# GEOS-ESM/QuickChem

Measured on NVIDIA B200. Metric: OH grid-cell predictions/sec, higher is better.
Workload: dtype f32

## Files before the change

### quickchem_b200/csrc/capi_xgb.cpp

```cpp
#include "context.hpp"

#include <condition_variable>
#include <mutex>
#ifdef __linux__
#include <sched.h>
#endif
#if defined(__x86_64__)
#include <emmintrin.h>
#endif

using namespace qcoh;

namespace qcoh {
template <class T>
static cudaTextureObject_t linear_texture(T *p, size_t n) {
  cudaResourceDesc rd;
  memset(&rd, 0, sizeof rd);
  rd.resType = cudaResourceTypeLinear;
  rd.res.linear.devPtr = p;
  rd.res.linear.desc = cudaCreateChannelDesc<T>();
  rd.res.linear.sizeInBytes = n * sizeof(T);
  cudaTextureDesc td;
  memset(&td, 0, sizeof td);
  td.readMode = cudaReadModeElementType;
  cudaTextureObject_t t = 0;
  CU(cudaCreateTextureObject(&t, &rd, &td, nullptr));
  return t;
}

void upload(Booster *b) {
  if (b->uploaded) return;
  if (!b->loaded) throw Error("Booster has no model: call XGBoosterLoadModel first");
  ensure_device();
  const FlatForest &f = b->flat;
  const size_t nn = (size_t)f.num_nodes();
  {
    std::vector<uint32_t> dev_nodes(f.nodes_xy);
    for (size_t i = 0; i < nn; ++i) {
      if ((dev_nodes[2 * i + 1] & kMetaRelMask) == 0) continue;
      float thr;
      memcpy(&thr, &dev_nodes[2 * i], 4);
      if (std::isnan(thr)) throw Error("split threshold is NaN (node " + std::to_string(i) + ")");
      dev_nodes[2 * i] = neg_threshold_key(thr);
    }
    CU(cudaMemcpy(b->d_nodes.need(nn), dev_nodes.data(), nn * 8, cudaMemcpyHostToDevice));
    b->dev_nodes_host = std::move(dev_nodes);
  }
  CU(cudaMemcpy(b->d_off.need(f.tree_offset.size()), f.tree_offset.data(), f.tree_offset.size() * 4, cudaMemcpyHostToDevice));
  {
    std::vector<int32_t> dd(f.tree_depth.size());
    for (size_t i = 0; i < dd.size(); ++i) {
      if (f.tree_depth[i] > 255) throw Error("tree " + std::to_string(i) + " is deeper than 255 levels");
      dd[i] = f.tree_depth[i] | (std::min(f.tree_min_leaf_depth[i], 255) << 8);
    }
    CU(cudaMemcpy(b->d_depth.need(dd.size()), dd.data(), dd.size() * 4, cudaMemcpyHostToDevice));
  }
  CU(cudaMemcpy(b->d_orig.need(nn), f.orig_id.data(), nn * 4, cudaMemcpyHostToDevice));
  if (b->dev.tex) cudaDestroyTextureObject(b->dev.tex);
  if (b->dev.tex4) cudaDestroyTextureObject(b->dev.tex4);
  b->dev = DeviceForest();
  b->dev.nodes = b->d_nodes.p, b->dev.tree_offset = b->d_off.p, b->dev.tree_depth = b->d_depth.p, b->dev.orig_id = b->d_orig.p;
  b->dev.ntree = (int32_t)b->host.trees.size();
  b->dev.nfeat = (int32_t)b->host.num_feature;
  b->dev.base_score = b->host.base_score;
  if (nn > 0 && nn < ((size_t)1 << 27)) b->dev.tex = linear_texture(b->d_nodes.p, nn);
  if (b->duo.ok && b->duo.num_slots() > 0 && b->duo.num_slots() < ((int64_t)1 << 27)) {
    const size_t ns = (size_t)b->duo.num_slots();
    CU(cudaMemcpy(b->d_recs.need(ns), b->duo.rec.data(), ns * 16, cudaMemcpyHostToDevice));
    b->dev.tex4 = linear_texture(b->d_recs.p, ns);
    b->dev.recs = b->d_recs.p;
    b->dev.duo_has_dl = b->duo.has_default_bits ? 1 : 0;
    b->dev.duo_shallow = (int64_t)ns * 16 < kShallowRecBytesPerTree * std::max<int64_t>(1, b->dev.ntree) ? 1 : 0;
    b->dev.duo_blk_mul = 1u << (32 - b->duo.blk_shift);
  }
  b->uploaded = true;
}

static thread_local struct {
  uint64_t owner = 0;
  ConstWindow w;
} g_const;

ConstWindow hold(Booster *b, int tree0, int ntree) {
  if (ntree <= 0 || ntree > kConstTreesMax || tree0 + ntree > b->dev.ntree) return {};
  int w0 = tree0 - tree0 % kConstTreesMax;
  if (tree0 + ntree > w0 + kConstTreesMax) w0 = tree0;
  const int n = std::min(b->dev.ntree - w0, kConstTreesMax);
  auto held = [&](TopLayout l) { return g_const.owner == b->version && g_const.w.holds(l, tree0, tree0 + ntree); };
  auto fill = [&](TopLayout l) {
    g_const.owner = 0;
    const cudaError_t e = l == TopLayout::kRecordTops
                              ? upload_const_duo(b->duo.top_xy.data() + (size_t)w0 * (2u << kDuoTop), b->duo.tree_slot.data() + w0, n, g.stream)
                              : upload_const_top(b->dev_nodes_host.data(), b->flat.tree_offset.data() + w0, n, g.stream);
    if (e != cudaSuccess) {
      (void)cudaGetLastError();
      return false;
    }
    g_const.owner = b->version, g_const.w = ConstWindow{l, w0, n};
    return true;
  };
  const bool records = b->dev.recs != nullptr && b->dev.tex != 0 && g.duo != 0;
  if (records && (held(TopLayout::kRecordTops) || fill(TopLayout::kRecordTops))) return g_const.w;
  if (held(TopLayout::kNodeTops) || fill(TopLayout::kNodeTops)) return g_const.w;
  return {};
}

void launch_predict_chunked(Booster *b, PredictArgs a, cudaStream_t s) {
  const int t_end = a.tree_end;
  if (a.nrow == 0) return;
  if (t_end <= 0) {
    if (!a.pred_leaf) {
      float v = b->host.base_score;
      if (a.exp10) v = (float)exp10((double)v) * a.scale;
      CU(launch_fill(a.out, a.nrow, v, s));
    }
    return;
  }
  for (int t0 = 0; t0 < t_end; t0 += kRangeTrees) {
    const int n = std::min(kRangeTrees, t_end - t0);
    const ConstWindow w = hold(b, t0, n);
    PredictArgs c = a;
    c.tree_begin = t0, c.tree_end = t0 + n;
    c.first = t0 == 0, c.last = t0 + n == t_end;
    CU(launch_predict(b->dev, w, c, s));
  }
}

static void seal(DMatrix *d) {
  ensure_device();
  int *fl = d->flags.need(1);
  CU(cudaMemsetAsync(fl, 0, sizeof(int), g.stream));
  if (g_spare_Xt.cap >= tile_words(d->nrow, d->ncol) && g_spare_Xt.p && !d->Xt.p) d->Xt.swap(g_spare_Xt);
  CU(launch_seal_tiles(d->X.p, d->nrow, (int)d->ncol, d->missing, d->Xt.need(tile_words(d->nrow, d->ncol)), fl, g.stream));
  CU(cudaMemcpyAsync(&d->hflags, fl, sizeof(int), cudaMemcpyDeviceToHost, g.stream));
  CU(cudaStreamSynchronize(g.stream));
  d->sealed = true;
  if (d->hflags & 2) throw Error("Check failed: valid: Input data contains `inf` or `nan`");
}

static unsigned trees_used(const Booster *b, unsigned ntree_limit) {
  const unsigned nt = (unsigned)b->host.trees.size();
  return (ntree_limit == 0 || ntree_limit > nt) ? nt : ntree_limit;
}

static void predict_into(Booster *b, DMatrix *d, int option_mask, unsigned ntree_limit, const qcoh_epilogue *epi, float *out_dev) {
  upload(b);
  if (!d->sealed) seal(d);
  if (option_mask & ~3) throw Error("option_mask " + std::to_string(option_mask) + ": only 0 (value), 1 (margin) and 2 (leaf index) are supported");
  if (d->ncol > b->host.num_feature)
    throw Error("Check failed: Number of columns does not match number of features in booster. Columns: " +
                std::to_string(d->ncol) + " Features: " + std::to_string(b->host.num_feature));
  PredictArgs a;
  a.Xt = d->Xt.p, a.nrow = d->nrow, a.ncol = (int32_t)d->ncol;
// ... 826 lines not shown
```

### quickchem_b200/csrc/context.hpp

```cpp
#pragma once
#include <cuda_runtime.h>
#include <nvtx3/nvToolsExt.h>

#include <algorithm>
#include <cmath>
#include <cstdio>
#include <cstdlib>
#include <cstring>
#include <memory>
#include <mutex>
#include <stdexcept>
#include <string>
#include <thread>
#include <unordered_set>
#include <utility>
#include <vector>

#include "../../include/qcoh.h"
#include "forest.hpp"
#include "kernels.hpp"

namespace qcoh {

inline thread_local std::string g_err;
// ... 99 lines not shown
}

template <class T>
struct DevBuf {
  T *p = nullptr;
  size_t cap = 0;
  T *need(size_t n) {
    if (n > cap) {
      if (p) cudaFree(p);
      p = nullptr, cap = 0;
      CU(cudaMalloc((void **)&p, (n ? n : 1) * sizeof(T)));
      cap = n;
    }
    return p;
  }
  void release() {
    if (p) cudaFree(p);
    p = nullptr, cap = 0;
  }
  void swap(DevBuf &o) {
    std::swap(p, o.p);
    std::swap(cap, o.cap);
  }
  DevBuf() = default;
  DevBuf(const DevBuf &) = delete;
  DevBuf &operator=(const DevBuf &) = delete;
  ~DevBuf() { release(); }
};

template <class T>
struct PinBuf {
  T *p = nullptr;
  size_t cap = 0;
  T *need(size_t n) {
    if (n > cap) {
      if (p) cudaFreeHost(p);
      p = nullptr, cap = 0;
      CU(cudaHostAlloc((void **)&p, (n ? n : 1) * sizeof(T), cudaHostAllocDefault));
      cap = n;
    }
    return p;
  }
  void swap(PinBuf &o) {
    std::swap(p, o.p);
    std::swap(cap, o.cap);
  }
  PinBuf() = default;
  PinBuf(const PinBuf &) = delete;
  PinBuf &operator=(const PinBuf &) = delete;
  ~PinBuf() {
    if (p) cudaFreeHost(p);
  }
};

inline bool is_device_ptr(const void *p) {
  cudaPointerAttributes a;
  cudaError_t e = cudaPointerGetAttributes(&a, p);
  if (e != cudaSuccess) {
    (void)cudaGetLastError();
    return false;
  }
  return a.type == cudaMemoryTypeDevice || a.type == cudaMemoryTypeManaged;
}

constexpr uint32_t kBoosterMagic = 0x51434253;
constexpr uint32_t kDMatrixMagic = 0x5143444d;
constexpr uint32_t kOhMagic = 0x51434f48;

inline thread_local std::unordered_set<const void *> g_live_handles;
inline bool is_live(const void *h) { return h && g_live_handles.count(h) != 0; }

struct Booster {
  uint32_t magic = kBoosterMagic;
  int oh_refs = 0;
  uint64_t version = 0;
  bool loaded = false, uploaded = false;
  bool cache_owned = false;
  HostForest host;
  FlatForest flat;
  std::vector<uint32_t> dev_nodes_host;
  DeviceForest dev;
  DuoForest duo;
  DevBuf<uint4> d_recs;
  DevBuf<uint2> d_nodes;
  DevBuf<uint32_t> d_off;
  DevBuf<int32_t> d_depth, d_orig;
  DevBuf<float> d_result;
  PinBuf<float> h_result;
  std::vector<bst_ulong> h_shape;
  ShapForest shap;
  bool shap_uploaded = false;
  DevBuf<uint4> d_shap_bins;
  DevBuf<float> d_shap_mean;
  DevBuf<double> d_shap_part;
  Booster() = default;
  Booster(const Booster &) = delete;
  Booster &operator=(const Booster &) = delete;
  ~Booster() {
    if (dev.tex) cudaDestroyTextureObject(dev.tex);
    if (dev.tex4) cudaDestroyTextureObject(dev.tex4);
  }
};

struct DMatrix {
  uint32_t magic = kDMatrixMagic;
  uint64_t nrow = 0, ncol = 0;
  float missing = NAN;
  DevBuf<float> X;
  DevBuf<uint32_t> Xt;
  DevBuf<int> flags;
  int hflags = 1;
  bool sealed = false;
  const void *spec_booster = nullptr;
  uint64_t spec_version = 0;
  bool spec_ready = false;
  DevBuf<float> spec_dev;
  PinBuf<float> spec_host;
};

inline thread_local DevBuf<float> g_spare_X;
inline thread_local DevBuf<uint32_t> g_spare_Xt;
inline thread_local PinBuf<float> g_spare_pin;
inline thread_local DevBuf<float> g_spare_spec;
inline thread_local DevBuf<int> g_chunk_flags;
inline thread_local PinBuf<int> g_h_chunk_flags;
inline thread_local Booster *g_last_booster = nullptr;
inline thread_local uint64_t g_version_counter = 0;

inline Booster *B(BoosterHandle h) {
  Booster *b = (Booster *)h;
  if (!b || !is_live(h) || b->magic != kBoosterMagic) throw Error("Invalid booster handle");
  return b;
}
inline DMatrix *D(DMatrixHandle h) {
  DMatrix *d = (DMatrix *)h;
  if (!d || !is_live(h) || d->magic != kDMatrixMagic) throw Error("Invalid DMatrix handle");
  return d;
}

void upload(Booster *b);
ConstWindow hold(Booster *b, int tree0, int ntree);
void launch_predict_chunked(Booster *b, PredictArgs a, cudaStream_t s);
const ShapForest &shap_tables(Booster *b);

}
```

### quickchem_b200/csrc/forest.hpp

```cpp
#pragma once
#include <cstdint>
#include <cstring>
#include <string>
#include <vector>

namespace qcoh {

struct HostTree {
  std::vector<int32_t> cleft, cright, parent;
  std::vector<uint32_t> sindex;
  std::vector<float> info;
  std::vector<float> loss_chg, sum_hess, base_weight;
  std::vector<int32_t> leaf_child_cnt;
  int32_t num_nodes() const { return (int32_t)cleft.size(); }
};

enum ModelFormat { kLegacyBinary = 0, kJson = 1, kUbjson = 2 };

struct HostForest {
  float base_score = 0.5f;
  uint32_t num_feature = 0;
  uint32_t version[3] = {1, 6, 0};
  std::string objective = "reg:squarederror";
  std::vector<HostTree> trees;
  std::vector<int32_t> tree_info;
  std::vector<std::pair<std::string, std::string>> attributes;
  ModelFormat format = kLegacyBinary;
};

constexpr uint32_t kMetaFeatShift = 26;
constexpr uint32_t kMetaDefaultLeftBit = 1u << 23;
constexpr uint32_t kMetaRelMask = (1u << 23) - 1;
constexpr uint32_t kMaxFeatures = 31;

struct FlatForest {
  std::vector<uint32_t> nodes_xy;
  std::vector<uint32_t> tree_offset;
  std::vector<int32_t> tree_depth;
  std::vector<int32_t> tree_min_leaf_depth;
  std::vector<int32_t> orig_id;
  int32_t max_depth = 0;
  int64_t num_nodes() const { return (int64_t)orig_id.size(); }
};

inline uint32_t neg_threshold_key(float thr) {
  thr += 0.0f;
  uint32_t bits;
  memcpy(&bits, &thr, 4);
  return 0u - (bits ^ ((bits >> 31) ? 0xFFFFFFFFu : 0x80000000u));
}

constexpr int kDuoTop = 4;
constexpr uint32_t kDuoDlRoot = 1u << 17, kDuoDlLeft = 1u << 16, kDuoDlRight = 1u << 15;
constexpr uint32_t kTopDefaultLeftBit = 1u;
struct DuoForest {
  bool ok = false;
  std::string why;
  int blk_shift = 18;
  bool has_default_bits = true;
  std::vector<uint32_t> rec;
  std::vector<uint32_t> tree_slot;
  std::vector<uint32_t> top_xy;
  int64_t num_slots() const { return (int64_t)(rec.size() / 4); }
};
DuoForest build_duo(const struct FlatForest &f, uint32_t num_feature);

constexpr uint32_t kShapNoFeature = 0xFF;
struct ShapForest {
  bool ok = false;
  std::vector<float> mean;
  std::vector<uint32_t> bins;
  std::vector<int64_t> tree_bin;
  int32_t max_path_len = 0;
  int64_t num_paths = 0, num_elements = 0;
  int64_t num_bins() const { return (int64_t)(bins.size() / 128); }
};
ShapForest build_shap(const struct HostForest &h, const struct FlatForest &f);
float shap_bias(const ShapForest &s, const struct HostForest &h, const struct FlatForest &f, int ntree);

struct PredictConfig {
  int type = 0;
  bool training = false;
  int64_t iteration_begin = 0, iteration_end = 0;
  bool strict_shape = false;
};
PredictConfig parse_predict_config(const char *json);

HostForest load_model_file(const std::string &path);
HostForest load_model_buffer(const unsigned char *buf, size_t len);
void save_model_file(const HostForest &f, const std::string &path);
FlatForest flatten(const HostForest &f);

}
```

### quickchem_b200/csrc/kernels.cu

```cuda
#include "kernels.hpp"

#include <cfloat>
#include <cmath>
#include <cstring>
#include <vector>

#include "forest.hpp"

namespace qcoh {

static thread_local uint64_t g_launches = 0;
uint64_t launch_count() { return g_launches; }

#define QC_LAUNCHED() (++g_launches, cudaGetLastError())

namespace {
enum Family { kDuo, kNodes8 = kDuo + 4, kSoaDuo = kNodes8 + 4, kSoaNodes8, kSealTiles, kShap, kShapReduce, kShapApprox, kFamilies };
const char *const kFamilyName[kFamilies] = {"duo", "duo_missing", "duo_leaf", "duo_missing_leaf", "nodes8", "nodes8_missing",
                                            "nodes8_leaf", "nodes8_missing_leaf", "soa_duo", "soa_nodes8", "seal_tiles",
                                            "shap", "shap_reduce", "shap_approx"};
thread_local uint64_t g_family[kFamilies];
thread_local const char *g_last_predict = "";
void count_family(int f) { ++g_family[f]; }
void count_predict(int f) { ++g_family[f], g_last_predict = kFamilyName[f]; }
}
uint64_t kernel_launches(const char *family) {
  for (int i = 0; i < kFamilies; ++i)
    if (!strcmp(kFamilyName[i], family)) return g_family[i];
  return 0;
}
const char *last_predict_kernel() { return g_last_predict; }

__global__ void fill_kernel(float *p, uint64_t n, float v) {
  const uint64_t stride = (uint64_t)gridDim.x * blockDim.x;
  for (uint64_t i = (uint64_t)blockIdx.x * blockDim.x + threadIdx.x; i < n; i += stride) p[i] = v;
}
cudaError_t launch_fill(float *p, uint64_t n, float v, cudaStream_t s) {
  if (n == 0) return cudaSuccess;
  int blocks = (int)((n + 255) / 256 < 148 * 16 ? (n + 255) / 256 : 148 * 16);
  fill_kernel<<<blocks, 256, 0, s>>>(p, n, v);
  return QC_LAUNCHED();
}

constexpr int kBlock = kTileRows;
constexpr int kStride = kTileRows;
static_assert(kStride * 4 == 1024, "the address arithmetic of the walks assumes a 1 KB feature stride");

constexpr uint32_t kKeyMissing = 0xFFFFFFFFu;
__device__ __forceinline__ uint32_t float_key(float v) {
  const uint32_t b = __float_as_uint(__fadd_rn(v, 0.0f));
  return b ^ ((uint32_t)((int32_t)b >> 31) | 0x80000000u);
}
__device__ __forceinline__ uint32_t step_index(uint32_t idx, uint32_t rel, uint32_t x, uint32_t kv) {
  asm("{\n\t.reg .u32 t;\n\tadd.cc.u32 t, %2, %3;\n\taddc.u32 %0, %0, %1;\n\t}" : "+r"(idx) : "r"(rel), "r"(x), "r"(kv));
  return idx;
}
__device__ __forceinline__ uint32_t add_carry_out(uint32_t a, uint32_t b) {
  uint32_t c;
  asm("{\n\t.reg .u32 t;\n\tadd.cc.u32 t, %1, %2;\n\taddc.u32 %0, 0, 0;\n\t}" : "=r"(c) : "r"(a), "r"(b));
  return c;
}
__device__ __forceinline__ uint32_t lds_u32(uint32_t saddr) {
  uint32_t v;
  asm volatile("ld.shared.u32 %0, [%1];" : "=r"(v) : "r"(saddr));
  return v;
}

constexpr int kConstTopNodes = kConstTreesMax << kDuoTop;
__constant__ uint2 c_top[kConstTopNodes];
__constant__ uint32_t c_duo_base[kConstTreesMax];

cudaError_t upload_const_top(const uint32_t *dev_nodes_xy, const uint32_t *tree_offset, int ntree, cudaStream_t s) {
  constexpr int stride = 1 << kDuoTop;
  if (ntree > kConstTreesMax) return cudaErrorInvalidValue;
  std::vector<uint2> host((size_t)ntree * stride);
  for (int t = 0; t < ntree; ++t) {
    const uint32_t n0 = tree_offset[t], n1 = tree_offset[t + 1];
    for (int i = 0; i < stride; ++i) {
      const uint32_t n = n0 + (uint32_t)i;
      host[t * stride + i] = n < n1 ? make_uint2(dev_nodes_xy[2 * n], dev_nodes_xy[2 * n + 1]) : make_uint2(0u, 0u);
    }
  }
  return cudaMemcpyToSymbolAsync(c_top, host.data(), sizeof(uint2) * (size_t)ntree * stride, 0, cudaMemcpyHostToDevice, s);
}

cudaError_t upload_const_duo(const uint32_t *top_xy, const uint32_t *tree_slot, int ntree, cudaStream_t s) {
  if (ntree > kConstTreesMax) return cudaErrorInvalidValue;
  cudaError_t e = cudaMemcpyToSymbolAsync(c_top, top_xy, sizeof(uint2) * ((size_t)ntree << kDuoTop), 0, cudaMemcpyHostToDevice, s);
  if (e != cudaSuccess) return e;
  return cudaMemcpyToSymbolAsync(c_duo_base, tree_slot, sizeof(uint32_t) * (size_t)ntree, 0, cudaMemcpyHostToDevice, s);
}

__device__ __forceinline__ void mbar_init(uint32_t bar, uint32_t count) {
  asm volatile("mbarrier.init.shared::cta.b64 [%0], %1;" ::"r"(bar), "r"(count));
}
__device__ __forceinline__ void mbar_init_fence() { asm volatile("fence.mbarrier_init.release.cluster;" ::: "memory"); }
__device__ __forceinline__ void mbar_expect_tx(uint32_t bar, uint32_t bytes) {
  asm volatile("mbarrier.arrive.expect_tx.shared::cta.b64 _, [%0], %1;" ::"r"(bar), "r"(bytes) : "memory");
}
__device__ __forceinline__ void bulk_g2s(uint32_t dst, const void *src, uint32_t bytes, uint32_t bar) {
  asm volatile("cp.async.bulk.shared::cluster.global.mbarrier::complete_tx::bytes [%0], [%1], %2, [%3];" ::"r"(dst),
               "l"(src), "r"(bytes), "r"(bar)
               : "memory");
}
__device__ __forceinline__ void mbar_wait(uint32_t bar, uint32_t parity) {
  asm volatile(
      "{\n"
      ".reg .pred p;\n"
      "WAIT_%=:\n"
      "mbarrier.try_wait.parity.shared::cta.b64 p, [%0], %1;\n"
      "@p bra DONE_%=;\n"
      "bra WAIT_%=;\n"
      "DONE_%=:\n"
      "}\n" ::"r"(bar),
      "r"(parity)
      : "memory");
}

struct TilePipe {
  uint32_t smem0, bar0, tile_bytes, src_skip, dst_skip;
  const uint32_t *Xt;
  uint64_t ntile, tile, tile_stride;
  uint32_t it;
  __device__ __forceinline__ void issue(uint64_t t) const {
    mbar_expect_tx(bar0, tile_bytes);
    if (tile_bytes) bulk_g2s(smem0 + dst_skip, Xt + t * tile_stride + src_skip, tile_bytes, bar0);
  }
  __device__ __forceinline__ void begin(uint32_t *smem, unsigned long long *bar, const PredictArgs &a, int nfeat, bool with_order, int tid) {
    smem0 = (uint32_t)__cvta_generic_to_shared(smem), bar0 = (uint32_t)__cvta_generic_to_shared(bar);
    tile_stride = (uint64_t)(a.ncol + 1) * kStride;
    tile_bytes = (uint32_t)(a.ncol + (with_order ? 1 : 0)) * kStride * 4u;
    src_skip = with_order ? 0u : (uint32_t)kStride, dst_skip = with_order ? 0u : (uint32_t)kStride * 4u;
    Xt = a.Xt, ntile = (a.nrow + kTileRows - 1) / kTileRows, tile = blockIdx.x, it = 0;
    uint32_t *k = smem + kStride;
    for (int c = a.ncol; c < nfeat; ++c) k[c * kStride + tid] = kKeyMissing;
    k[nfeat * kStride + tid] = 0u;
    if (tid == 0) {
      mbar_init(bar0, 1);
      mbar_init_fence();
    }
    __syncthreads();
    if (tid == 0 && tile < ntile) issue(tile);
  }
  __device__ __forceinline__ bool more() const { return tile < ntile; }
  __device__ __forceinline__ uint32_t acquire(int tid) {
    if (tid == 0) mbar_wait(bar0, it & 1u);
    __syncthreads();
// ... 94 lines not shown
    minleaf = min(minleaf, dd >> 8);
    nd[j] = make_uint2(0u, 0u);
    rel[j] = 1u;
  }
  auto visit = [&](int j) {
    static_assert(kMetaFeatShift == 26, "address trick assumes feat in the top 6 bits");
    const uint32_t kv = lds_u32(my_saddr + __byte_perm(nd[j].y, 0u, 0x4434));
    rel[j] = nd[j].y & kMetaRelMask;
    if (HAS_MISSING && kv == kKeyMissing)
      idx[j] += rel[j] + ((nd[j].y & kMetaDefaultLeftBit) ? 0u : (rel[j] != 0u ? 1u : 0u));
    else
      idx[j] = step_index(idx[j], rel[j], nd[j].x, kv);
  };
  if (CTOP > 0) {
    uint32_t cbase[ILP];
#pragma unroll
    for (int j = 0; j < ILP; ++j) cbase[j] = ((uint32_t)(t + j - ctree0) << CTOP) - idx[j];
    if (minleaf >= CTOP) {
#pragma unroll
      for (int d = 0; d < CTOP; ++d) {
#pragma unroll
        for (int j = 0; j < ILP; ++j) {
          nd[j] = c_top[cbase[j] + idx[j]];
          visit(j);
        }
      }
    } else {
#pragma unroll
      for (int d = 0; d < CTOP; ++d) {
        if (d <= depth) {
#pragma unroll
          for (int j = 0; j < ILP; ++j) {
            if (rel[j] != 0u) {
              nd[j] = c_top[cbase[j] + idx[j]];
              visit(j);
            }
            asm volatile("" : "+r"(rel[j]));
          }
        }
      }
    }
  }
  auto fetch = [&](int j) {
    if ((TEXMODE >> j) & 1)
      nd[j] = tex1Dfetch<uint2>(tex, (int)idx[j]);
    else
      nd[j] = __ldg(nodes + idx[j]);
  };
  for (int d = CTOP; d < depth; ++d) {
#pragma unroll
    for (int j = 0; j < ILP; ++j) {
      if (rel[j] != 0u) {
        fetch(j);
        visit(j);
      }
      asm volatile("" : "+r"(rel[j]));
    }
  }
  if (depth >= CTOP) {
#pragma unroll
    for (int j = 0; j < ILP; ++j)
      if (rel[j] != 0u) fetch(j);
  }
#pragma unroll
  for (int j = 0; j < ILP; ++j) xbits[j] = nd[j].x;
}

template <int ILP, bool HAS_MISSING, int TEXMODE, int CTOP, class Emit>
__device__ __forceinline__ void forest_walk(const DeviceForest &f, uint32_t my, int ctree0, int t0, int t1, Emit &&emit) {
  int t = t0;
  for (; t + ILP <= t1; t += ILP) {
    uint32_t idx[ILP], xb[ILP];
    walk_group<ILP, HAS_MISSING, TEXMODE, CTOP>(f.nodes, f.tex, f.tree_offset, f.tree_depth, t, ctree0, my, idx, xb);
#pragma unroll
    for (int j = 0; j < ILP; ++j) emit(t + j, xb[j], idx[j]);
  }
  for (; t < t1; ++t) {
    uint32_t idx[1], xb[1];
    walk_group<1, HAS_MISSING, 0, 0>(f.nodes, f.tex, f.tree_offset, f.tree_depth, t, 0, my, idx, xb);
    emit(t, xb[0], idx[0]);
  }
}

template <int ILP, int TEXMODE, bool HAS_MISSING>
__device__ __forceinline__ void walk_group_duo(const uint4 *__restrict__ recs, cudaTextureObject_t tex4,
                                               const int32_t *__restrict__ tdepth, uint32_t blk_mul, int t, int ctree0, uint32_t my_saddr,
                                               uint32_t (&xbits)[ILP], uint32_t (&ids)[ILP]) {
  constexpr int CTOP = kDuoTop;
  int depth = CTOP - 1;
  uint32_t idx[ILP];
#pragma unroll
  for (int j = 0; j < ILP; ++j) {
    depth = max(depth, __ldg(tdepth + t + j) & 0xFF);
    idx[j] = 1u;
  }
  const int tl = t - ctree0;
#pragma unroll
  for (int d = 0; d < CTOP; ++d) {
#pragma unroll
    for (int j = 0; j < ILP; ++j) {
      const uint2 nd = c_top[((uint32_t)(tl + j) << CTOP) + idx[j]];
      const uint32_t kv = lds_u32(my_saddr + __byte_perm(nd.y, 0u, 0x4434));
      if (HAS_MISSING) {
        uint32_t right = add_carry_out(nd.x, kv);
        if (kv == kKeyMissing) right = (nd.y & kTopDefaultLeftBit) ^ 1u;
        idx[j] = 2u * idx[j] + right;
      } else {
        idx[j] = step_index(idx[j], idx[j], nd.x, kv);
      }
    }
  }
  uint4 r[ILP];
  uint32_t walking[ILP];
#pragma unroll
  for (int j = 0; j < ILP; ++j) {
    idx[j] += c_duo_base[tl + j] - (1u << CTOP);
    r[j] = make_uint4(0u, 0u, 0u, 0u);
    walking[j] = 1u;
  }
  auto gather = [&](int j) {
    if (walking[j] != 0u) {
      if ((TEXMODE >> j) & 1)
        r[j] = tex1Dfetch<uint4>(tex4, (int)idx[j]);
      else
        r[j] = __ldg(recs + idx[j]);
    }
  };
  int d = CTOP;
  for (; d + 2 <= depth + 1; d += 2) {
#pragma unroll
    for (int j = 0; j < ILP; ++j) gather(j);
    uint32_t kv0[ILP], kv[ILP], right1[ILP];
#pragma unroll
    for (int j = 0; j < ILP; ++j) {
      uint32_t sa;
      asm("mad.lo.u32 %0, %1, %2, %3;" : "=r"(sa) : "r"(r[j].w & 31u), "r"((uint32_t)(kStride * 4)), "r"(my_saddr));
      kv0[j] = lds_u32(sa);
    }
#pragma unroll
    for (int j = 0; j < ILP; ++j) {
      right1[j] = add_carry_out(r[j].x, kv0[j]);
      if (HAS_MISSING && kv0[j] == kKeyMissing) right1[j] = (r[j].w & kDuoDlRoot) ? 0u : 1u;
      const uint32_t ms = right1[j] ? (r[j].w << 5) : r[j].w;
      kv[j] = lds_u32(my_saddr + (ms & (31u << 10)));
    }
#pragma unroll
    for (int j = 0; j < ILP; ++j) {
      const uint32_t xs = right1[j] ? r[j].z : r[j].y;
      uint32_t blk;
      asm("mul.hi.u32 %0, %1, %2;" : "=r"(blk) : "r"(r[j].w), "r"(blk_mul));
      if (HAS_MISSING) {
        uint32_t right2 = add_carry_out(xs, kv[j]);
        if (kv[j] == kKeyMissing) right2 = (r[j].w & (right1[j] ? kDuoDlRight : kDuoDlLeft)) ? 0u : 1u;
        const uint32_t half = 2u * blk + right1[j];
        idx[j] = c_duo_base[tl + j] + 2u * half + right2;
      } else {
        uint32_t half;
        asm("{\n\t.reg .u32 t;\n\tadd.cc.u32 t, %1, %2;\n\tmadc.lo.u32 %0, %3, 2, 0;\n\t}" : "=r"(half) : "r"(r[j].x), "r"(kv0[j]), "r"(blk));
        idx[j] = step_index(c_duo_base[tl + j] + half, half, xs, kv[j]);
      }
      walking[j] = blk;
      asm volatile("" : "+r"(walking[j]));
    }
  }
#pragma unroll
  for (int j = 0; j < ILP; ++j) gather(j);
#pragma unroll
  for (int j = 0; j < ILP; ++j) xbits[j] = r[j].x, ids[j] = r[j].y;
}

template <int ILP, int TEXMODE, bool HAS_MISSING, class Emit>
__device__ __forceinline__ void forest_walk_duo(const DeviceForest &f, uint32_t my, int ctree0, int t0, int t1, Emit &&emit) {
  int t = t0;
  for (; t + ILP <= t1; t += ILP) {
    uint32_t xb[ILP], id[ILP];
    walk_group_duo<ILP, TEXMODE, HAS_MISSING>(f.recs, f.tex4, f.tree_depth, f.duo_blk_mul, t, ctree0, my, xb, id);
#pragma unroll
    for (int j = 0; j < ILP; ++j) emit(t + j, xb[j], id[j]);
  }
  constexpr int H = ILP / 2;
  if (H >= 2) {
    for (; t + H <= t1; t += H) {
      uint32_t xb[H > 0 ? H : 1], id[H > 0 ? H : 1];
      walk_group_duo<(H > 0 ? H : 1), ((1 << H) - 2), HAS_MISSING>(f.recs, f.tex4, f.tree_depth, f.duo_blk_mul, t, ctree0, my, xb, id);
#pragma unroll
      for (int j = 0; j < H; ++j) emit(t + j, xb[j], id[j]);
    }
  }
  for (; t < t1; ++t) {
    uint32_t xb[1], id[1];
    walk_group_duo<1, 0, HAS_MISSING>(f.recs, f.tex4, f.tree_depth, f.duo_blk_mul, t, ctree0, my, xb, id);
    emit(t, xb[0], id[0]);
  }
}

template <int ILP, int TEXMASK, int MINB>
struct DuoWalk {
  static constexpr int kMinBlocks = MINB, kFamily = kDuo;
  __device__ static bool walks_missing(const DeviceForest &f) { return f.duo_has_dl != 0; }
  template <bool HAS_MISSING, bool PRED_LEAF, class Emit>
  __device__ __forceinline__ static void run(const DeviceForest &f, uint32_t my, int ctree0, int t0, int t1, Emit &&emit) {
    forest_walk_duo<ILP, TEXMASK, HAS_MISSING>(f, my, ctree0, t0, t1, emit);
  }
};
template <int ILP, int TEXMASK, int CTOP, int MINB>
struct NodesWalk {
  static constexpr int kMinBlocks = MINB, kFamily = kNodes8;
  __device__ static bool walks_missing(const DeviceForest &) { return true; }
  template <bool HAS_MISSING, bool PRED_LEAF, class Emit>
  __device__ __forceinline__ static void run(const DeviceForest &f, uint32_t my, int ctree0, int t0, int t1, Emit &&emit) {
    forest_walk<ILP, HAS_MISSING, TEXMASK, CTOP>(f, my, ctree0, t0, t1, [&](int t, uint32_t xb, uint32_t idx) {
      emit(t, xb, PRED_LEAF ? (uint32_t)__ldg(f.orig_id + idx) : 0u);
    });
  }
};

using RecordsWalk = DuoWalk<6, 0x36, 5>;
using RecordsShallowWalk = DuoWalk<4, 0xA, 6>;
using NodesTableWalk = NodesWalk<4, 0xA, kDuoTop, 6>;
using NodesTexWalk = NodesWalk<4, 0xA, 0, 6>;
using NodesLsuWalk = NodesWalk<4, 0, 0, 6>;

__device__ __forceinline__ float export_transform(float acc, int exp10_on, float scale) {
  if (!exp10_on) return acc;
  const float p = (float)exp10((double)acc);
  return __fmul_rn(p, scale);
}

template <bool PRED_LEAF, class Walk>
__device__ __forceinline__ void row_result(const DeviceForest &f, const PredictArgs &a, uint64_t row, bool live, Walk &&walk) {
  if (PRED_LEAF) {
    float *o = a.out + row * (uint64_t)a.out_stride;
    walk([&](int t, uint32_t, uint32_t id) {
      if (live) o[t] = (float)id;
    });
  } else {
    float acc = f.base_score;
    if (!a.first && live) acc = a.out[row];
    walk([&](int, uint32_t xb, uint32_t) { acc = __fadd_rn(acc, __uint_as_float(xb)); });
    if (live) a.out[row] = a.last ? export_transform(acc, a.exp10, a.scale) : acc;
  }
}

template <bool HAS_MISSING>
__device__ __forceinline__ uint64_t tile_row(uint32_t buf, uint64_t tile, int tid, bool absent_columns, bool &hm) {
  uint32_t orig = (uint32_t)tid;
  hm = false;
  if (HAS_MISSING) {
    const uint32_t p = lds_u32(buf + 4u * (uint32_t)tid);
    orig = p & 0xFFu;
    hm = __any_sync(0xffffffffu, (p >> 8) & 1u) || absent_columns;
  }
  return tile * kTileRows + orig;
}

template <class Walk, bool HAS_MISSING, bool PRED_LEAF>
__global__ void __launch_bounds__(kBlock, Walk::kMinBlocks) predict_tiles_kernel(DeviceForest f, PredictArgs a) {
  extern __shared__ __align__(128) uint32_t skey[];
  __shared__ __align__(8) unsigned long long bars[1];
  const int tid = threadIdx.x;
  TilePipe pipe;
  pipe.begin(skey, bars, a, f.nfeat, HAS_MISSING, tid);
  while (pipe.more()) {
    const uint32_t buf = pipe.acquire(tid);
    const uint32_t my = buf + 4u * (uint32_t)(kStride + tid);
    bool hm;
    const uint64_t row = tile_row<HAS_MISSING>(buf, pipe.tile, tid, a.ncol < f.nfeat, hm);
    row_result<PRED_LEAF>(f, a, row, row < a.nrow, [&](auto &&emit) {
      if (HAS_MISSING && hm)
        Walk::template run<true, PRED_LEAF>(f, my, a.ctree0, a.tree_begin, a.tree_end, emit);
      else
        Walk::template run<false, PRED_LEAF>(f, my, a.ctree0, a.tree_begin, a.tree_end, emit);
    });
    pipe.release(tid);
  }
}

template <class Walk, class MissingWalk>
__global__ void __launch_bounds__(kBlock, Walk::kMinBlocks) predict_soa_kernel(DeviceForest f, SoaArgs a) {
  extern __shared__ __align__(128) uint32_t skey[];
  const int tid = threadIdx.x;
  constexpr int B = kBlock;
  const uint64_t m = (uint64_t)blockIdx.x * B + tid;
  const bool live = m < a.nrow;
  int flags = 0;
  if (live) {
    const size_t e = a.e0 + m;
    const int c = (int)(m % (uint64_t)a.ncol);
    const bool chk_inf = !isinf(a.missing);
#pragma unroll
    for (int ft = 0; ft < 27; ++ft) {
      float x;
      if (ft == 1)
        x = __fdiv_rn(__fmul_rn(__fadd_rn(__ldg(a.ple + e), __ldg(a.ple + e + a.ncol)), 0.5f), 100.0f);
      else
        x = a.src3[ft] ? __ldg(a.src3[ft] + e) : __ldg(a.src2[ft] + c);
      uint32_t k = float_key(x);
      if (x != x || x == a.missing) k = kKeyMissing, flags |= 1;
      if (chk_inf && isinf(x)) flags |= 2;
      skey[ft * kStride + tid] = k;
    }
  } else {
#pragma unroll
    for (int ft = 0; ft < 27; ++ft) skey[ft * kStride + tid] = 0u;
  }
  skey[27 * kStride + tid] = 0u;
  const bool tile_missing = __syncthreads_or(flags & 1) != 0;
  if (__syncthreads_or(flags & 2) != 0) {
    if (tid == 0) atomicOr(a.flags, 2);
  }
  if (!live) return;
  const uint32_t my = (uint32_t)__cvta_generic_to_shared(skey + tid);
  float acc = f.base_score;
  auto add = [&](int, uint32_t xb, uint32_t) { acc = __fadd_rn(acc, __uint_as_float(xb)); };
  if (!tile_missing || Walk::walks_missing(f)) {
    if (tile_missing)
      Walk::template run<true, false>(f, my, a.ctree0, 0, a.ntree_used, add);
    else
      Walk::template run<false, false>(f, my, a.ctree0, 0, a.ntree_used, add);
  } else {
    MissingWalk::template run<true, false>(f, my, a.ctree0, 0, a.ntree_used, add);
  }
  if (a.pred) a.pred[m] = acc;
  a.out[m] = export_transform(acc, a.exp10, a.scale);
}

enum class Layout { kRecords, kNodesTable, kNodesTex, kNodesLsu };
static Layout layout(const DeviceForest &f, const ConstWindow &w, int t0, int t1, bool has_missing) {
  if (w.holds(TopLayout::kRecordTops, t0, t1) && (!has_missing || f.duo_has_dl)) return Layout::kRecords;
  if (f.tex == 0) return Layout::kNodesLsu;
  return w.holds(TopLayout::kNodeTops, t0, t1) ? Layout::kNodesTable : Layout::kNodesTex;
}

cudaError_t launch_predict_soa(const DeviceForest &f, const ConstWindow &w, const SoaArgs &args, cudaStream_t s) {
  if (args.nrow == 0) return cudaSuccess;
  if (f.nfeat != 27) return cudaErrorInvalidValue;
  const size_t smem = (size_t)kStride * 28 * sizeof(float);
  const uint64_t nblk = (args.nrow + kBlock - 1) / kBlock;
  if (nblk > 0x7fffffffull) return cudaErrorInvalidConfiguration;
  SoaArgs a = args;
  a.ctree0 = w.tree0;
  const Layout l = layout(f, w, 0, a.ntree_used, false);
  auto k = predict_soa_kernel<RecordsWalk, NodesTexWalk>;
  if (l == Layout::kNodesTable) k = predict_soa_kernel<NodesTableWalk, NodesTableWalk>;
  if (l == Layout::kNodesTex) k = predict_soa_kernel<NodesTexWalk, NodesTexWalk>;
  if (l == Layout::kNodesLsu) k = predict_soa_kernel<NodesLsuWalk, NodesLsuWalk>;
  cudaError_t e = cudaFuncSetAttribute(k, cudaFuncAttributeMaxDynamicSharedMemorySize, (int)smem);
  if (e != cudaSuccess) return e;
  k<<<dim3((unsigned)nblk), kBlock, smem, s>>>(f, a);
  count_family(l == Layout::kRecords ? kSoaDuo : kSoaNodes8);
  return QC_LAUNCHED();
}

static thread_local int g_sm_count = 0;
static int sm_count() {
  if (g_sm_count == 0) {
    int dev = 0;
    cudaGetDevice(&dev);
    if (cudaDeviceGetAttribute(&g_sm_count, cudaDevAttrMultiProcessorCount, dev) != cudaSuccess || g_sm_count <= 0) g_sm_count = 148;
  }
  return g_sm_count;
}

template <class K>
static cudaError_t launch_tiles(K k, const DeviceForest &f, const PredictArgs &a, cudaStream_t s) {
  const size_t smem = (size_t)kStride * (size_t)(f.nfeat + 2) * sizeof(uint32_t);
  const uint64_t grid = tile_count(a.nrow);
  if (grid > 0x7fffffffull) return cudaErrorInvalidConfiguration;
  cudaError_t e = cudaFuncSetAttribute(k, cudaFuncAttributeMaxDynamicSharedMemorySize, (int)smem);
  if (e != cudaSuccess) return e;
  k<<<dim3((unsigned)grid), kBlock, smem, s>>>(f, a);
  return QC_LAUNCHED();
}

template <class Walk>
static cudaError_t launch_walk(const DeviceForest &f, const PredictArgs &a, cudaStream_t s) {
  const bool hm = a.has_missing != 0, pl = a.pred_leaf != 0;
  count_predict(Walk::kFamily + hm + 2 * pl);
  if (hm && pl) return launch_tiles(predict_tiles_kernel<Walk, true, true>, f, a, s);
  if (hm) return launch_tiles(predict_tiles_kernel<Walk, true, false>, f, a, s);
  if (pl) return launch_tiles(predict_tiles_kernel<Walk, false, true>, f, a, s);
  return launch_tiles(predict_tiles_kernel<Walk, false, false>, f, a, s);
}

cudaError_t launch_predict(const DeviceForest &f, const ConstWindow &w, const PredictArgs &args, cudaStream_t s) {
  if (args.nrow == 0 || args.tree_end <= args.tree_begin) return cudaSuccess;
  if (args.ncol > f.nfeat || f.nfeat > (int)kMaxFeatures) return cudaErrorInvalidValue;
  PredictArgs a = args;
  a.ctree0 = w.tree0;
  switch (layout(f, w, a.tree_begin, a.tree_end, a.has_missing != 0)) {
    case Layout::kRecords: return f.duo_shallow ? launch_walk<RecordsShallowWalk>(f, a, s) : launch_walk<RecordsWalk>(f, a, s);
    case Layout::kNodesTable: return launch_walk<NodesTableWalk>(f, a, s);
    case Layout::kNodesTex: return launch_walk<NodesTexWalk>(f, a, s);
    case Layout::kNodesLsu: break;
  }
  return launch_walk<NodesLsuWalk>(f, a, s);
}

constexpr unsigned kFull = 0xffffffffu;

__device__ __forceinline__ int shap_region_words(int nf) {
  const int ast = nf | 1;
  return max(2 * kTileRows * ast, kTileRows * (nf + 2));
}

__global__ void __launch_bounds__(kTileRows, 2) shap_paths_kernel(const uint4 *__restrict__ bins, int64_t nbins, int nslices,
                                                                  ContribArgs a, double *__restrict__ part) {
  extern __shared__ __align__(128) uint32_t smem[];
  __shared__ __align__(8) unsigned long long bars[1];
  __shared__ double s_inv[34];
  const int nf = a.nfeat, tid = threadIdx.x, lane = tid & 31, warp = tid >> 5;
  const int ast = nf | 1, kst = nf | 1;
  double *acc = reinterpret_cast<double *>(smem);
  uint32_t *keys = smem + shap_region_words(nf);
  uint32_t *order = keys + kTileRows * kst;
  PredictArgs pa;
  pa.Xt = a.Xt, pa.nrow = a.nrow, pa.ncol = a.ncol;
  TilePipe pipe;
  pipe.begin(smem, bars, pa, nf, true, tid);
  if (tid < 34) s_inv[tid] = tid ? 1.0 / (double)tid : 0.0;
  (void)pipe.acquire(tid);
  order[tid] = smem[tid];
  for (int c = 0; c < nf; ++c) keys[tid * kst + c] = smem[(1 + c) * kStride + tid];
  __syncthreads();
  for (int i = tid; i < kTileRows * ast; i += kTileRows) acc[i] = 0.0;
  __syncthreads();
  const uint64_t tile = blockIdx.x;
  const int64_t b0 = nbins * (int64_t)blockIdx.y / nslices, b1 = nbins * (int64_t)(blockIdx.y + 1) / nslices;
  for (int64_t b = b0; b < b1; ++b) {
    const uint4 e = __ldg(bins + b * 32 + lane);
    const uint32_t feat = e.z & 0xFFu, g0 = (e.z >> 16) & 31u, len = e.z >> 24;
    const int j = lane - (int)g0, D = (int)len - 1;
    const bool elem = feat != kShapNoFeature && j >= 1;
    const bool miss_here = (e.z >> 8) & 1u;
    const float zf = __uint_as_float(e.w);
    const double z = elem ? (double)zf : 1.0;
    const double v = (double)__shfl_sync(kFull, zf, (int)g0);
    const int maxlen = (int)__reduce_max_sync(kFull, len);
    const double invz = 1.0 / z, d1 = (double)(D + 1), inv_d1 = s_inv[D + 1 > 0 ? D + 1 : 0];
    const unsigned starts = __ballot_sync(kFull, len > 0 && j == 0);
    const int ngroups = __popc(starts), my_group = __popc(starts & ((1u << g0) - 1u));
    for (int r = warp * 32; r < warp * 32 + 32; ++r) {
      const uint32_t orig = order[r] & 0xFFu;
      if (tile * kTileRows + orig >= a.nrow) continue;
      bool one = true;
      if (elem) {
        const uint32_t k = keys[r * kst + feat];
        one = k == kKeyMissing ? miss_here : (e.x <= k && k < e.y);
      }
      const float zo = one ? zf : -zf;
      double pw = j == 0 ? 1.0 : 0.0;
      for (int i = 1; i < maxlen; ++i) {
        const float zi = __shfl_sync(kFull, zo, (int)(g0 + i) & 31);
        const double left = __shfl_up_sync(kFull, pw, 1);
        if (i <= D) {
          const double inv = s_inv[i + 1];
          pw = (double)fabsf(zi) * pw * (double)max(i - j, 0) * inv + (zi > 0.f ? left : 0.0) * (double)j * inv;
        }
      }
      double next = __shfl_sync(kFull, pw, (int)(g0 + (D > 0 ? D : 0)) & 31), total = 0.0;
      for (int i = maxlen - 2; i >= 0; --i) {
        const double pwi = __shfl_sync(kFull, pw, (int)(g0 + min(i, D > 0 ? D : 0)) & 31);
        if (i < D) {
          if (one) {
            const double tmp = next * d1 * s_inv[i + 1];
// ... 342 lines not shown
```

### quickchem_b200/csrc/kernels.hpp

```cpp
#pragma once
#include <cuda_runtime.h>

#include <cstdint>

namespace qcoh {

struct DeviceForest {
  const uint2 *nodes = nullptr;
  const uint32_t *tree_offset = nullptr;
  const int32_t *tree_depth = nullptr;
  const int32_t *orig_id = nullptr;
  cudaTextureObject_t tex = 0;
  const uint4 *recs = nullptr;
  cudaTextureObject_t tex4 = 0;
  int duo_has_dl = 0;
  uint32_t duo_blk_mul = 0;
  int32_t ntree = 0;
  int32_t nfeat = 0;
  int duo_shallow = 0;
  float base_score = 0.f;
};

enum class TopLayout { kNone, kRecordTops, kNodeTops };
struct ConstWindow {
  TopLayout layout = TopLayout::kNone;
  int32_t tree0 = 0, ntree = 0;
  bool holds(TopLayout l, int t0, int t1) const { return layout == l && tree0 <= t0 && t1 <= tree0 + ntree; }
};

constexpr int kConstTreesMax = 480;
constexpr int kRangeTrees = 120;
constexpr int64_t kShallowRecBytesPerTree = 4096;

constexpr int kTileRows = 256;
constexpr uint64_t kMaxMatrixCols = 192;
inline uint64_t tile_count(uint64_t nrow) { return (nrow + kTileRows - 1) / kTileRows; }
inline size_t tile_words(uint64_t nrow, uint64_t ncol) { return (size_t)tile_count(nrow) * (size_t)(ncol + 1) * kTileRows; }
inline size_t tile_offset_words(uint64_t row0, uint64_t ncol) { return (size_t)(row0 / kTileRows) * (size_t)(ncol + 1) * kTileRows; }

struct PredictArgs {
  const uint32_t *Xt = nullptr;
  uint64_t nrow = 0;
  int32_t ncol = 0;
  int has_missing = 1;
  int pred_leaf = 0;
  int32_t tree_begin = 0;
  int32_t tree_end = 0;
  int32_t out_stride = 0;
  int first = 1;
  int last = 1;
  int exp10 = 0;
  float scale = 1.f;
  float *out = nullptr;
  int32_t ctree0 = 0;
};

uint64_t launch_count();
uint64_t kernel_launches(const char *family);
const char *last_predict_kernel();

cudaError_t upload_const_top(const uint32_t *dev_nodes_xy, const uint32_t *tree_offset, int ntree, cudaStream_t s);
cudaError_t upload_const_duo(const uint32_t *top_xy, const uint32_t *tree_slot, int ntree, cudaStream_t s);

cudaError_t launch_seal_tiles(const float *X, uint64_t nrow, int ncol, float missing, uint32_t *Xt, int *flags, cudaStream_t s);

cudaError_t launch_predict(const DeviceForest &f, const ConstWindow &w, const PredictArgs &a, cudaStream_t s);

constexpr int kShapSlices = 16;
constexpr uint64_t kShapChunkRows = 32768;
struct ContribArgs {
  const uint32_t *Xt = nullptr;
  uint64_t nrow = 0;
  int32_t ncol = 0;
  int32_t nfeat = 0;
  float bias = 0.f;
  float *out = nullptr;
};
cudaError_t launch_shap(const uint4 *bins, int64_t nbins, int nslices, const ContribArgs &a, double *part, cudaStream_t s);
cudaError_t launch_shap_reduce(const double *part, int nslices, const ContribArgs &a, cudaStream_t s);
cudaError_t launch_shap_approx(const DeviceForest &f, const float *mean, int ntree, const ContribArgs &a, cudaStream_t s);

struct SoaArgs {
  const float *src3[27];
  const float *src2[27];
  const float *ple = nullptr;
  int32_t ncol = 0;
  uint64_t e0 = 0;
  uint64_t nrow = 0;
  float missing = -999.f;
  int32_t ntree_used = 0;
  int32_t ctree0 = 0;
  int exp10 = 1;
  float scale = 1.f;
  float *out = nullptr;
  float *pred = nullptr;
  int *flags = nullptr;
// ... 37 lines not shown
```

Measured before the change: 1.405 billion.

## Stage level-4 duo records in shared memory for the tiled records walk

Builds a per-tree compact array of the 16 level-4 records at upload time and copies the slice for the current tree range into shared memory at kernel start. The first record gather after the constant-memory top levels then reads shared memory instead of a global or texture fetch. This costs extra dynamic shared memory per block (16 records of 16 bytes per tree), and min blocks drops from 5 to 4. The fused SoA kernel keeps the old walk through a separate alias.

```diff
diff --git a/quickchem_b200/csrc/capi_xgb.cpp b/quickchem_b200/csrc/capi_xgb.cpp
--- a/quickchem_b200/csrc/capi_xgb.cpp
+++ b/quickchem_b200/csrc/capi_xgb.cpp
@@ -69,6 +69,11 @@
     CU(cudaMemcpy(b->d_recs.need(ns), b->duo.rec.data(), ns * 16, cudaMemcpyHostToDevice));
     b->dev.tex4 = linear_texture(b->d_recs.p, ns);
     b->dev.recs = b->d_recs.p;
+    std::vector<uint32_t> r4((size_t)b->dev.ntree * kDuoLevelRecs * 4);
+    for (int t = 0; t < b->dev.ntree; ++t)
+      memcpy(&r4[(size_t)t * kDuoLevelRecs * 4], &b->duo.rec[(size_t)b->duo.tree_slot[t] * 4], kDuoLevelRecs * 16);
+    CU(cudaMemcpy(b->d_recs4.need(r4.size() / 4), r4.data(), r4.size() * 4, cudaMemcpyHostToDevice));
+    b->dev.recs4 = b->d_recs4.p;
     b->dev.duo_has_dl = b->duo.has_default_bits ? 1 : 0;
     b->dev.duo_shallow = (int64_t)ns * 16 < kShallowRecBytesPerTree * std::max<int64_t>(1, b->dev.ntree) ? 1 : 0;
     b->dev.duo_blk_mul = 1u << (32 - b->duo.blk_shift);
diff --git a/quickchem_b200/csrc/context.hpp b/quickchem_b200/csrc/context.hpp
--- a/quickchem_b200/csrc/context.hpp
+++ b/quickchem_b200/csrc/context.hpp
@@ -205,6 +205,7 @@
   DeviceForest dev;
   DuoForest duo;
   DevBuf<uint4> d_recs;
+  DevBuf<uint4> d_recs4;
   DevBuf<uint2> d_nodes;
   DevBuf<uint32_t> d_off;
   DevBuf<int32_t> d_depth, d_orig;
diff --git a/quickchem_b200/csrc/forest.hpp b/quickchem_b200/csrc/forest.hpp
--- a/quickchem_b200/csrc/forest.hpp
+++ b/quickchem_b200/csrc/forest.hpp
@@ -51,6 +51,7 @@
 }
 
 constexpr int kDuoTop = 4;
+constexpr uint32_t kDuoLevelRecs = 1u << kDuoTop;
 constexpr uint32_t kDuoDlRoot = 1u << 17, kDuoDlLeft = 1u << 16, kDuoDlRight = 1u << 15;
 constexpr uint32_t kTopDefaultLeftBit = 1u;
 struct DuoForest {
diff --git a/quickchem_b200/csrc/kernels.cu b/quickchem_b200/csrc/kernels.cu
--- a/quickchem_b200/csrc/kernels.cu
+++ b/quickchem_b200/csrc/kernels.cu
@@ -63,6 +63,11 @@
 __device__ __forceinline__ uint32_t lds_u32(uint32_t saddr) {
   uint32_t v;
   asm volatile("ld.shared.u32 %0, [%1];" : "=r"(v) : "r"(saddr));
+  return v;
+}
+__device__ __forceinline__ uint4 lds_u128(uint32_t saddr) {
+  uint4 v;
+  asm volatile("ld.shared.v4.u32 {%0, %1, %2, %3}, [%4];" : "=r"(v.x), "=r"(v.y), "=r"(v.z), "=r"(v.w) : "r"(saddr));
   return v;
 }
 
@@ -323,10 +328,10 @@
   }
 }
 
-template <int ILP, int TEXMODE, bool HAS_MISSING>
+template <int ILP, int TEXMODE, bool HAS_MISSING, bool REC4>
 __device__ __forceinline__ void walk_group_duo(const uint4 *__restrict__ recs, cudaTextureObject_t tex4,
                                                const int32_t *__restrict__ tdepth, uint32_t blk_mul, int t, int ctree0, uint32_t my_saddr,
-                                               uint32_t (&xbits)[ILP], uint32_t (&ids)[ILP]) {
+                                               uint32_t rec4_saddr, uint32_t (&xbits)[ILP], uint32_t (&ids)[ILP]) {
   constexpr int CTOP = kDuoTop;
   int depth = CTOP - 1;
   uint32_t idx[ILP];
@@ -352,9 +357,10 @@
     }
   }
   uint4 r[ILP];
-  uint32_t walking[ILP];
+  uint32_t walking[ILP], rec4[ILP];
 #pragma unroll
   for (int j = 0; j < ILP; ++j) {
+    if (REC4) rec4[j] = rec4_saddr + 16u * (kDuoLevelRecs * (uint32_t)j + idx[j] - (1u << CTOP));
     idx[j] += c_duo_base[tl + j] - (1u << CTOP);
     r[j] = make_uint4(0u, 0u, 0u, 0u);
     walking[j] = 1u;
@@ -367,10 +373,21 @@
         r[j] = __ldg(recs + idx[j]);
     }
   };
+  auto first = [&](int j) {
+    if (REC4)
+      r[j] = lds_u128(rec4[j]);
+    else
+      gather(j);
+  };
   int d = CTOP;
   for (; d + 2 <= depth + 1; d += 2) {
 #pragma unroll
-    for (int j = 0; j < ILP; ++j) gather(j);
+    for (int j = 0; j < ILP; ++j) {
+      if (d == CTOP)
+        first(j);
+      else
+        gather(j);
+    }
     uint32_t kv0[ILP], kv[ILP], right1[ILP];
 #pragma unroll
     for (int j = 0; j < ILP; ++j) {
@@ -405,17 +422,23 @@
     }
   }
 #pragma unroll
-  for (int j = 0; j < ILP; ++j) gather(j);
+  for (int j = 0; j < ILP; ++j) {
+    if (d == CTOP)
+      first(j);
+    else
+      gather(j);
+  }
 #pragma unroll
   for (int j = 0; j < ILP; ++j) xbits[j] = r[j].x, ids[j] = r[j].y;
 }
 
-template <int ILP, int TEXMODE, bool HAS_MISSING, class Emit>
-__device__ __forceinline__ void forest_walk_duo(const DeviceForest &f, uint32_t my, int ctree0, int t0, int t1, Emit &&emit) {
+template <int ILP, int TEXMODE, bool HAS_MISSING, bool REC4, class Emit>
+__device__ __forceinline__ void forest_walk_duo(const DeviceForest &f, uint32_t my, uint32_t rec4, int ctree0, int t0, int t1, Emit &&emit) {
+  auto rec4_of = [&](int t) { return rec4 + (uint32_t)(t - t0) * (kDuoLevelRecs * 16u); };
   int t = t0;
   for (; t + ILP <= t1; t += ILP) {
     uint32_t xb[ILP], id[ILP];
-    walk_group_duo<ILP, TEXMODE, HAS_MISSING>(f.recs, f.tex4, f.tree_depth, f.duo_blk_mul, t, ctree0, my, xb, id);
+    walk_group_duo<ILP, TEXMODE, HAS_MISSING, REC4>(f.recs, f.tex4, f.tree_depth, f.duo_blk_mul, t, ctree0, my, rec4_of(t), xb, id);
 #pragma unroll
     for (int j = 0; j < ILP; ++j) emit(t + j, xb[j], id[j]);
   }
@@ -423,40 +446,44 @@
   if (H >= 2) {
     for (; t + H <= t1; t += H) {
       uint32_t xb[H > 0 ? H : 1], id[H > 0 ? H : 1];
-      walk_group_duo<(H > 0 ? H : 1), ((1 << H) - 2), HAS_MISSING>(f.recs, f.tex4, f.tree_depth, f.duo_blk_mul, t, ctree0, my, xb, id);
+      walk_group_duo<(H > 0 ? H : 1), ((1 << H) - 2), HAS_MISSING, REC4>(f.recs, f.tex4, f.tree_depth, f.duo_blk_mul, t, ctree0, my,
+                                                                          rec4_of(t), xb, id);
 #pragma unroll
       for (int j = 0; j < H; ++j) emit(t + j, xb[j], id[j]);
     }
   }
   for (; t < t1; ++t) {
     uint32_t xb[1], id[1];
-    walk_group_duo<1, 0, HAS_MISSING>(f.recs, f.tex4, f.tree_depth, f.duo_blk_mul, t, ctree0, my, xb, id);
+    walk_group_duo<1, 0, HAS_MISSING, REC4>(f.recs, f.tex4, f.tree_depth, f.duo_blk_mul, t, ctree0, my, rec4_of(t), xb, id);
     emit(t, xb[0], id[0]);
   }
 }
 
-template <int ILP, int TEXMASK, int MINB>
+template <int ILP, int TEXMASK, int MINB, bool REC4 = false>
 struct DuoWalk {
   static constexpr int kMinBlocks = MINB, kFamily = kDuo;
+  static constexpr bool kRec4 = REC4;
   __device__ static bool walks_missing(const DeviceForest &f) { return f.duo_has_dl != 0; }
   template <bool HAS_MISSING, bool PRED_LEAF, class Emit>
-  __device__ __forceinline__ static void run(const DeviceForest &f, uint32_t my, int ctree0, int t0, int t1, Emit &&emit) {
-    forest_walk_duo<ILP, TEXMASK, HAS_MISSING>(f, my, ctree0, t0, t1, emit);
+  __device__ __forceinline__ static void run(const DeviceForest &f, uint32_t my, uint32_t rec4, int ctree0, int t0, int t1, Emit &&emit) {
+    forest_walk_duo<ILP, TEXMASK, HAS_MISSING, REC4>(f, my, rec4, ctree0, t0, t1, emit);
   }
 };
 template <int ILP, int TEXMASK, int CTOP, int MINB>
 struct NodesWalk {
   static constexpr int kMinBlocks = MINB, kFamily = kNodes8;
+  static constexpr bool kRec4 = false;
   __device__ static bool walks_missing(const DeviceForest &) { return true; }
   template <bool HAS_MISSING, bool PRED_LEAF, class Emit>
-  __device__ __forceinline__ static void run(const DeviceForest &f, uint32_t my, int ctree0, int t0, int t1, Emit &&emit) {
+  __device__ __forceinline__ static void run(const DeviceForest &f, uint32_t my, uint32_t, int ctree0, int t0, int t1, Emit &&emit) {
     forest_walk<ILP, HAS_MISSING, TEXMASK, CTOP>(f, my, ctree0, t0, t1, [&](int t, uint32_t xb, uint32_t idx) {
       emit(t, xb, PRED_LEAF ? (uint32_t)__ldg(f.orig_id + idx) : 0u);
     });
   }
 };
 
-using RecordsWalk = DuoWalk<6, 0x36, 5>;
+using RecordsWalk = DuoWalk<6, 0x36, 4, true>;
+using RecordsSoaWalk = DuoWalk<6, 0x36, 5>;
 using RecordsShallowWalk = DuoWalk<4, 0xA, 6>;
 using NodesTableWalk = NodesWalk<4, 0xA, kDuoTop, 6>;
 using NodesTexWalk = NodesWalk<4, 0xA, 0, 6>;
@@ -500,6 +527,13 @@
   extern __shared__ __align__(128) uint32_t skey[];
   __shared__ __align__(8) unsigned long long bars[1];
   const int tid = threadIdx.x;
+  uint32_t rec4 = 0;
+  if (Walk::kRec4) {
+    uint4 *s4 = reinterpret_cast<uint4 *>(skey + (f.nfeat + 2) * kStride);
+    const uint4 *g4 = f.recs4 + (size_t)a.tree_begin * kDuoLevelRecs;
+    for (int i = tid; i < (a.tree_end - a.tree_begin) * (int)kDuoLevelRecs; i += kBlock) s4[i] = __ldg(g4 + i);
+    rec4 = (uint32_t)__cvta_generic_to_shared(s4);
+  }
   TilePipe pipe;
   pipe.begin(skey, bars, a, f.nfeat, HAS_MISSING, tid);
   while (pipe.more()) {
@@ -509,9 +543,9 @@
     const uint64_t row = tile_row<HAS_MISSING>(buf, pipe.tile, tid, a.ncol < f.nfeat, hm);
     row_result<PRED_LEAF>(f, a, row, row < a.nrow, [&](auto &&emit) {
       if (HAS_MISSING && hm)
-        Walk::template run<true, PRED_LEAF>(f, my, a.ctree0, a.tree_begin, a.tree_end, emit);
+        Walk::template run<true, PRED_LEAF>(f, my, rec4, a.ctree0, a.tree_begin, a.tree_end, emit);
       else
-        Walk::template run<false, PRED_LEAF>(f, my, a.ctree0, a.tree_begin, a.tree_end, emit);
+        Walk::template run<false, PRED_LEAF>(f, my, rec4, a.ctree0, a.tree_begin, a.tree_end, emit);
     });
     pipe.release(tid);
   }
@@ -519,6 +553,7 @@
 
 template <class Walk, class MissingWalk>
 __global__ void __launch_bounds__(kBlock, Walk::kMinBlocks) predict_soa_kernel(DeviceForest f, SoaArgs a) {
+  static_assert(!Walk::kRec4 && !MissingWalk::kRec4, "the fused kernel does not stage level-4 records");
   extern __shared__ __align__(128) uint32_t skey[];
   const int tid = threadIdx.x;
   constexpr int B = kBlock;
@@ -556,11 +591,11 @@
   auto add = [&](int, uint32_t xb, uint32_t) { acc = __fadd_rn(acc, __uint_as_float(xb)); };
   if (!tile_missing || Walk::walks_missing(f)) {
     if (tile_missing)
-      Walk::template run<true, false>(f, my, a.ctree0, 0, a.ntree_used, add);
+      Walk::template run<true, false>(f, my, 0u, a.ctree0, 0, a.ntree_used, add);
     else
-      Walk::template run<false, false>(f, my, a.ctree0, 0, a.ntree_used, add);
+      Walk::template run<false, false>(f, my, 0u, a.ctree0, 0, a.ntree_used, add);
   } else {
-    MissingWalk::template run<true, false>(f, my, a.ctree0, 0, a.ntree_used, add);
+    MissingWalk::template run<true, false>(f, my, 0u, a.ctree0, 0, a.ntree_used, add);
   }
   if (a.pred) a.pred[m] = acc;
   a.out[m] = export_transform(acc, a.exp10, a.scale);
@@ -582,7 +617,7 @@
   SoaArgs a = args;
   a.ctree0 = w.tree0;
   const Layout l = layout(f, w, 0, a.ntree_used, false);
-  auto k = predict_soa_kernel<RecordsWalk, NodesTexWalk>;
+  auto k = predict_soa_kernel<RecordsSoaWalk, NodesTexWalk>;
   if (l == Layout::kNodesTable) k = predict_soa_kernel<NodesTableWalk, NodesTableWalk>;
   if (l == Layout::kNodesTex) k = predict_soa_kernel<NodesTexWalk, NodesTexWalk>;
   if (l == Layout::kNodesLsu) k = predict_soa_kernel<NodesLsuWalk, NodesLsuWalk>;
@@ -604,8 +639,8 @@
 }
 
 template <class K>
-static cudaError_t launch_tiles(K k, const DeviceForest &f, const PredictArgs &a, cudaStream_t s) {
-  const size_t smem = (size_t)kStride * (size_t)(f.nfeat + 2) * sizeof(uint32_t);
+static cudaError_t launch_tiles(K k, const DeviceForest &f, const PredictArgs &a, size_t extra_smem, cudaStream_t s) {
+  const size_t smem = (size_t)kStride * (size_t)(f.nfeat + 2) * sizeof(uint32_t) + extra_smem;
   const uint64_t grid = tile_count(a.nrow);
   if (grid > 0x7fffffffull) return cudaErrorInvalidConfiguration;
   cudaError_t e = cudaFuncSetAttribute(k, cudaFuncAttributeMaxDynamicSharedMemorySize, (int)smem);
@@ -617,11 +652,12 @@
 template <class Walk>
 static cudaError_t launch_walk(const DeviceForest &f, const PredictArgs &a, cudaStream_t s) {
   const bool hm = a.has_missing != 0, pl = a.pred_leaf != 0;
+  const size_t x = Walk::kRec4 ? (size_t)(a.tree_end - a.tree_begin) * kDuoLevelRecs * sizeof(uint4) : 0;
   count_predict(Walk::kFamily + hm + 2 * pl);
-  if (hm && pl) return launch_tiles(predict_tiles_kernel<Walk, true, true>, f, a, s);
-  if (hm) return launch_tiles(predict_tiles_kernel<Walk, true, false>, f, a, s);
-  if (pl) return launch_tiles(predict_tiles_kernel<Walk, false, true>, f, a, s);
-  return launch_tiles(predict_tiles_kernel<Walk, false, false>, f, a, s);
+  if (hm && pl) return launch_tiles(predict_tiles_kernel<Walk, true, true>, f, a, x, s);
+  if (hm) return launch_tiles(predict_tiles_kernel<Walk, true, false>, f, a, x, s);
+  if (pl) return launch_tiles(predict_tiles_kernel<Walk, false, true>, f, a, x, s);
+  return launch_tiles(predict_tiles_kernel<Walk, false, false>, f, a, x, s);
 }
 
 cudaError_t launch_predict(const DeviceForest &f, const ConstWindow &w, const PredictArgs &args, cudaStream_t s) {
diff --git a/quickchem_b200/csrc/kernels.hpp b/quickchem_b200/csrc/kernels.hpp
--- a/quickchem_b200/csrc/kernels.hpp
+++ b/quickchem_b200/csrc/kernels.hpp
@@ -12,6 +12,7 @@
   const int32_t *orig_id = nullptr;
   cudaTextureObject_t tex = 0;
   const uint4 *recs = nullptr;
+  const uint4 *recs4 = nullptr;
   cudaTextureObject_t tex4 = 0;
   int duo_has_dl = 0;
   uint32_t duo_blk_mul = 0;
```

Measured after the change: 1.010 billion (median of 6 runs). -28.1%, worse.
